# PKU-EPIC/GAPartNet

Hardware: AMD Instinct MI355X
Metric: point-clouds/sec (20k pts, train step) (higher is better)
Workload: dtype f32

## Files before the change

gapartnet_amd/csrc/bn.hip:

```cpp
#include <cstdlib>

#include "bn_stats.h"
#include "gpn_common.h"

namespace {

typedef float f32x4 __attribute__((ext_vector_type(4)));
constexpr int kThreads = 256;
constexpr int kMaxBlocks = 128;


template <int T>
__device__ __forceinline__ double column_total(const double (*red)[T][4], int q, int c, int C4, int R, int part, int P) {
  double acc = 0.0;
  const int cc4 = c >> 2, j = c & 3;
  for (int rr = part; rr < R; rr += P) acc += red[q][rr * C4 + cc4][j];
  for (int off = P >> 1; off >= 1; off >>= 1) acc += __shfl_down(acc, off, P);
  return acc;
}

__host__ __device__ __forceinline__ int sub_lanes(int pairs, int T) {
  int P = 16;
  while (P > 1 && pairs * P > T) P >>= 1;
  return P;
// ... 166 lines not shown
    reinterpret_cast<f32x4*>(y)[t] = v;
  }
}

__global__ void bn_apply_eval_kernel(const gpn::BnFwdPtrs pa, const gpn::BnFwdPtrs pb, int64_t total4, int C4, float eps, int relu,
                                     const int64_t* __restrict__ n_dev) {
  const gpn::BnFwdPtrs& p = blockIdx.y ? pb : pa;
  if (n_dev) total4 = gpn::live_rows(n_dev, total4 / C4) * C4;
  if (blockIdx.x == 0 && p.invstd)
    for (int c = threadIdx.x; c < 4 * C4; c += blockDim.x) p.invstd[c] = 1.0f / sqrtf(p.running_var[c] + eps);
  for (int64_t t = (int64_t)blockIdx.x * blockDim.x + threadIdx.x; t < total4; t += (int64_t)gridDim.x * blockDim.x) {
    const int c4 = (int)(t % C4);
    const f32x4 mu = reinterpret_cast<const f32x4*>(p.running_mean)[c4], var = reinterpret_cast<const f32x4*>(p.running_var)[c4];
    f32x4 is;
#pragma unroll
    for (int j = 0; j < 4; ++j) is[j] = 1.0f / sqrtf(var[j] + eps);
    const f32x4 w = reinterpret_cast<const f32x4*>(p.weight)[c4], b = reinterpret_cast<const f32x4*>(p.bias)[c4];
    f32x4 v = (reinterpret_cast<const f32x4*>(p.x)[t] - mu) * is * w + b;
    if (p.res) v += reinterpret_cast<const f32x4*>(p.res)[t];
    if (relu) {
#pragma unroll
      for (int j = 0; j < 4; ++j) v[j] = v[j] > 0.f ? v[j] : 0.f;
    }
    reinterpret_cast<f32x4*>(p.y)[t] = v;
  }
}

__global__ __launch_bounds__(64) void bn_finalize_bwd_kernel(const double* __restrict__ partial, int blocks, int C,
                                                             float* __restrict__ dweight, float* __restrict__ dbias) {
  const int c = blockIdx.x;
  double s, ss;
  sum_partials(partial, blocks, C, c, s, ss);
  if (threadIdx.x != 0) return;
  dbias[c] = (float)s;
  dweight[c] = (float)ss;
}

__global__ void bn_apply_bwd_kernel(const float* __restrict__ x, const float* __restrict__ y, const float* __restrict__ dy,
                                    const float* __restrict__ mean, const float* __restrict__ invstd,
                                    const float* __restrict__ weight, const float* __restrict__ dweight,
                                    const float* __restrict__ dbias, int64_t total4, int C4, float inv_n, int relu,
                                    int training, float* __restrict__ dx, float* __restrict__ dres) {
  for (int64_t t = (int64_t)blockIdx.x * blockDim.x + threadIdx.x; t < total4; t += (int64_t)gridDim.x * blockDim.x) {
    const int c4 = (int)(t % C4);
    const f32x4 mu = reinterpret_cast<const f32x4*>(mean)[c4], is = reinterpret_cast<const f32x4*>(invstd)[c4];
    const f32x4 w = reinterpret_cast<const f32x4*>(weight)[c4];
    f32x4 g = reinterpret_cast<const f32x4*>(dy)[t];
    if (relu) {
      const f32x4 yv = reinterpret_cast<const f32x4*>(y)[t];
#pragma unroll
      for (int j = 0; j < 4; ++j) g[j] = yv[j] > 0.f ? g[j] : 0.f;
    }
    if (dres) reinterpret_cast<f32x4*>(dres)[t] = g;
    f32x4 v = g;
    if (training) {
      const f32x4 dw = reinterpret_cast<const f32x4*>(dweight)[c4], db = reinterpret_cast<const f32x4*>(dbias)[c4];
      const f32x4 xhat = (reinterpret_cast<const f32x4*>(x)[t] - mu) * is;
      v = g - db * inv_n - xhat * (dw * inv_n);
    }
    reinterpret_cast<f32x4*>(dx)[t] = v * is * w;
  }
}

constexpr int kApplyBatch = 4;

template <bool FIXED>
__global__ __launch_bounds__(kApplyThreads) void bn_apply_fwd_fold_kernel(gpn::BnFwdPtrs pa, gpn::BnFwdPtrs pb, int blocks, int64_t N,
                                                                         int64_t total4, int C4, float eps, float momentum,
                                                                         int relu, const int64_t* __restrict__ n_dev) {
  if (n_dev) {
    N = gpn::live_rows(n_dev, N);
    total4 = N * C4;
    if (N == 0) return;
  }
  const gpn::BnFwdPtrs& pp = blockIdx.y ? pb : pa;
  const float* __restrict__ x = pp.x;
  const float* __restrict__ res = pp.res;
  const void* __restrict__ partial = pp.partial;
  const float* __restrict__ weight = pp.weight;
  const float* __restrict__ bias = pp.bias;
  float* __restrict__ y = pp.y;
  float* __restrict__ mean = pp.mean;
  float* __restrict__ invstd = pp.invstd;
  float* __restrict__ running_mean = pp.running_mean;
  float* __restrict__ running_var = pp.running_var;
  __shared__ double red[2][FIXED ? 1 : kApplyThreads][4];
  __shared__ unsigned long long words[FIXED ? 4 : 1][FIXED ? kFoldMaxC : 1];
  __shared__ double sums[2][kFoldMaxC];
  __shared__ __attribute__((aligned(16))) float stat[4][kFoldMaxC];
  constexpr int U = kApplyBatch;
  const int C = C4 * 4;
  const int64_t stride = (int64_t)gridDim.x * kApplyThreads;
  const int step = (int)(stride % C4);
  int64_t t = (int64_t)blockIdx.x * kApplyThreads + threadIdx.x;
  int c4 = (int)(t % C4);
  f32x4 xv[U], rv[U];
#pragma unroll
  for (int k = 0; k < U; ++k) {
    const int64_t tt = t + k * stride;
    if (tt < total4) {
      xv[k] = reinterpret_cast<const f32x4*>(x)[tt];
      if (res) rv[k] = reinterpret_cast<const f32x4*>(res)[tt];
    }
  }
  if constexpr (FIXED)
    fold_fixed<false>(static_cast<const unsigned long long*>(partial), C, blocks, reinterpret_cast<unsigned long long (*)[kFoldMaxC]>(&words[0][0]), sums);
  else
    fold_partials(static_cast<const double*>(partial), blocks, C4, reinterpret_cast<double (*)[kApplyThreads][4]>(&red[0][0][0]), sums);
  for (int c = threadIdx.x; c < C; c += kApplyThreads) {
    const double m = sums[0][c] / (double)N;
    double var = sums[1][c] / (double)N - m * m;
    if (var < 0.0) var = 0.0;
    const float mu = (float)m, is = (float)(1.0 / sqrt(var + (double)eps));
    stat[0][c] = mu;
    stat[1][c] = is;
    stat[2][c] = weight[c];
    stat[3][c] = bias[c];
    if (blockIdx.x == 0) {
      mean[c] = mu;
      invstd[c] = is;
      if (running_mean) {
        const double unbiased = N > 1 ? var * ((double)N / (double)(N - 1)) : var;
        running_mean[c] = (float)((1.0 - momentum) * running_mean[c] + momentum * m);
        running_var[c] = (float)((1.0 - momentum) * running_var[c] + momentum * unbiased);
      }
    }
  }
  __syncthreads();
  while (true) {
#pragma unroll
    for (int k = 0; k < U; ++k) {
      const int64_t tt = t + k * stride;
      if (tt < total4) {
        const f32x4 mu = reinterpret_cast<const f32x4*>(stat[0])[c4], is = reinterpret_cast<const f32x4*>(stat[1])[c4];
        const f32x4 w = reinterpret_cast<const f32x4*>(stat[2])[c4], b = reinterpret_cast<const f32x4*>(stat[3])[c4];
        f32x4 v = (xv[k] - mu) * is * w + b;
        if (res) v += rv[k];
        if (relu) {
#pragma unroll
          for (int j = 0; j < 4; ++j) v[j] = v[j] > 0.f ? v[j] : 0.f;
        }
        reinterpret_cast<f32x4*>(y)[tt] = v;
      }
      c4 += step;
      c4 = c4 >= C4 ? c4 - C4 : c4;
    }
    t += U * stride;
    if (t >= total4) break;
#pragma unroll
    for (int k = 0; k < U; ++k) {
      const int64_t tt = t + k * stride;
      if (tt < total4) {
        xv[k] = reinterpret_cast<const f32x4*>(x)[tt];
        if (res) rv[k] = reinterpret_cast<const f32x4*>(res)[tt];
      }
    }
  }
}

template <bool FIXED>
__global__ __launch_bounds__(kApplyThreads) void bn_apply_bwd_fold_kernel(gpn::BnBwdPtrs pa, gpn::BnBwdPtrs pb, int blocks, int64_t total4,
                                                                         int C4, float inv_n, int relu, int training,
                                                                         const int64_t* __restrict__ n_dev) {
  if (n_dev) {
    const int64_t N = gpn::live_rows(n_dev, total4 / C4);
    total4 = N * C4;
    inv_n = 1.0f / (float)N;
    if (N == 0) {
      if (blockIdx.x == 0) {
        const gpn::BnBwdPtrs& q = blockIdx.y ? pb : pa;
        for (int c = threadIdx.x; c < C4 * 4; c += kApplyThreads) q.dbias[c] = 0.f, q.dweight[c] = 0.f;
      }
      return;
    }
  }
  const gpn::BnBwdPtrs& pp = blockIdx.y ? pb : pa;
  const float* __restrict__ x = pp.x;
  const float* __restrict__ y = pp.y;
  const float* __restrict__ dy = pp.dy;
  const void* __restrict__ partial = pp.partial;
  const float* __restrict__ mean = pp.mean;
  const float* __restrict__ invstd = pp.invstd;
  const float* __restrict__ weight = pp.weight;
  float* __restrict__ dx = pp.dx;
  float* __restrict__ dres = pp.dres;
  float* __restrict__ dweight = pp.dweight;
  float* __restrict__ dbias = pp.dbias;
  __shared__ double red[2][FIXED ? 1 : kApplyThreads][4];
  __shared__ unsigned long long words[FIXED ? 4 : 1][FIXED ? kFoldMaxC : 1];
  __shared__ double sums[2][kFoldMaxC];
  __shared__ __attribute__((aligned(16))) float stat[5][kFoldMaxC];
  constexpr int U = kApplyBatch;
  const int C = C4 * 4;
  const int64_t stride = (int64_t)gridDim.x * kApplyThreads;
  const int step = (int)(stride % C4);
  int64_t t = (int64_t)blockIdx.x * kApplyThreads + threadIdx.x;
  int c4 = (int)(t % C4);
  f32x4 gv[U], yv[U], xv[U];
#pragma unroll
  for (int k = 0; k < U; ++k) {
    const int64_t tt = t + k * stride;
    if (tt < total4) {
      gv[k] = reinterpret_cast<const f32x4*>(dy)[tt];
      if (relu) yv[k] = reinterpret_cast<const f32x4*>(y)[tt];
      if (training) xv[k] = reinterpret_cast<const f32x4*>(x)[tt];
    }
  }
  if constexpr (FIXED)
    fold_fixed<true>(static_cast<const unsigned long long*>(partial), C, blocks, reinterpret_cast<unsigned long long (*)[kFoldMaxC]>(&words[0][0]), sums);
  else
    fold_partials(static_cast<const double*>(partial), blocks, C4, reinterpret_cast<double (*)[kApplyThreads][4]>(&red[0][0][0]), sums);
  for (int c = threadIdx.x; c < C; c += kApplyThreads) {
    const float db = (float)sums[0][c], dw = (float)sums[1][c];
    stat[0][c] = db;
    stat[1][c] = dw;
    stat[2][c] = mean[c];
    stat[3][c] = invstd[c];
    stat[4][c] = weight[c];
    if (blockIdx.x == 0) {
      dbias[c] = db;
      dweight[c] = dw;
    }
  }
  __syncthreads();
  while (true) {
#pragma unroll
    for (int k = 0; k < U; ++k) {
      const int64_t tt = t + k * stride;
// ... 3 lines not shown
        if (relu) {
#pragma unroll
          for (int j = 0; j < 4; ++j) g[j] = yv[k][j] > 0.f ? g[j] : 0.f;
        }
        if (dres) reinterpret_cast<f32x4*>(dres)[tt] = g;
        f32x4 v = g;
        if (training) {
          const f32x4 db = reinterpret_cast<const f32x4*>(stat[0])[c4], dw = reinterpret_cast<const f32x4*>(stat[1])[c4];
          const f32x4 mu = reinterpret_cast<const f32x4*>(stat[2])[c4];
          const f32x4 xhat = (xv[k] - mu) * is;
          v = g - db * inv_n - xhat * (dw * inv_n);
        }
        reinterpret_cast<f32x4*>(dx)[tt] = v * is * w;
      }
      c4 += step;
      c4 = c4 >= C4 ? c4 - C4 : c4;
    }
    t += U * stride;
    if (t >= total4) break;
#pragma unroll
    for (int k = 0; k < U; ++k) {
      const int64_t tt = t + k * stride;
      if (tt < total4) {
        gv[k] = reinterpret_cast<const f32x4*>(dy)[tt];
        if (relu) yv[k] = reinterpret_cast<const f32x4*>(y)[tt];
        if (training) xv[k] = reinterpret_cast<const f32x4*>(x)[tt];
      }
    }
  }
}

constexpr int kSmallRows = 1024;

template <int CG, int T>
__device__ __forceinline__ void column_sum8(double (&v)[8], double (*scratch)[CG][8] ) {
  constexpr int W = T / 64;
#pragma unroll
  for (int off = 32; off >= CG; off >>= 1) {
#pragma unroll
    for (int q = 0; q < 8; ++q) v[q] += __shfl_down(v[q], off, 64);
  }
  if ((threadIdx.x & 63) < CG) {
#pragma unroll
    for (int q = 0; q < 8; ++q) scratch[threadIdx.x >> 6][threadIdx.x & 63][q] = v[q];
  }
  __syncthreads();
  const int cg = threadIdx.x % CG;
#pragma unroll
  for (int q = 0; q < 8; ++q) {
// ... 104 lines not shown
    reinterpret_cast<f32x4*>(dbias)[c4] = db;
    reinterpret_cast<f32x4*>(dweight)[c4] = dw;
  }
  const f32x4 w = reinterpret_cast<const f32x4*>(weight)[c4];
  const float inv_n = 1.0f / (float)N;
#pragma unroll 8
  for (int row = rl; row < N; row += R) {
    const int64_t t = (int64_t)row * C4 + c4;
    f32x4 g = reinterpret_cast<const f32x4*>(dy)[t];
    if (relu) {
      const f32x4 yv = reinterpret_cast<const f32x4*>(y)[t];
#pragma unroll
      for (int j = 0; j < 4; ++j) g[j] = yv[j] > 0.f ? g[j] : 0.f;
    }
    if (dres) reinterpret_cast<f32x4*>(dres)[t] = g;
    f32x4 v = g;
    if (training) {
      const f32x4 xhat = (reinterpret_cast<const f32x4*>(x)[t] - mu) * is;
      v = g - db * inv_n - xhat * (dw * inv_n);
    }
    reinterpret_cast<f32x4*>(dx)[t] = v * is * w;
  }
}

int reduce_blocks(int64_t N, int C4) {
  const int R = kReduceThreads / C4;
  int64_t b = gpn::cdiv(N, (int64_t)R * 2);
  if (b > kMaxBlocks) b = kMaxBlocks;
  if (b < 1) b = 1;
  return (int)b;
}

int fold_grid(int64_t total4) {
  int64_t g = gpn::cdiv(total4, (int64_t)kApplyThreads);
  if (g > 320) g = 320;
  return (int)(g < 1 ? 1 : g);
}

constexpr size_t kReduceLds = (size_t)2 * kReduceThreads * 4 * sizeof(double);

int apply_grid(int64_t total4) {
  int64_t g = gpn::cdiv(total4, kThreads);
  if (g > 4096) g = 4096;
  return (int)(g < 1 ? 1 : g);
}

// ... 144 lines not shown
  hipLaunchKernelGGL(bn_finalize_bwd_kernel, dim3(C), dim3(64), 0, stream, partial, blocks, C,
                     dweight, dbias);
  GPN_CHECK_LAUNCH();
  hipLaunchKernelGGL(bn_apply_bwd_kernel, dim3(apply_grid(total4)), dim3(kThreads), 0, stream, x, y, dy, mean, invstd,
                     weight, dweight, dbias, total4, C4, 1.0f / (float)N, relu, training, dx, dres);
  GPN_CHECK_LAUNCH();
  return GPN_OK;
}

bool gpn::bn_two_pass(int64_t N, int C) { return N >= 1 && C % 4 == 0 && C <= kFoldMaxC; }

int gpn::bn_fwd_train_fused(const gpn::BnFwdPtrs& p, const gpn::BnFwdPtrs* twin, int64_t N, int C, float eps, float momentum,
                            int relu, hipStream_t stream, const gpn::DevRows& rows) {
  for (const gpn::BnFwdPtrs* q : {&p, twin}) {
    if (!q) continue;
    GPN_CHECK_ARG(q->x && q->weight && q->bias && q->y && q->mean && q->invstd && q->partial);
    GPN_CHECK_ARG((q->running_mean == nullptr) == (q->running_var == nullptr));
  }
  GPN_CHECK_ARG(gpn::bn_two_pass(N, C));
  GPN_CHECK_ARG(!twin || (twin->res == nullptr) == (p.res == nullptr));
  const int64_t total4 = N * (C / 4);
  gpn::ProfScope prof(GPN_K_BN, stream, 0.0, 4.0 * (double)N * C * (p.res ? 3 : 2) * (twin ? 2 : 1), rows.dev, N);
  const int64_t Np = gpn::plan_rows(N, rows);
  hipLaunchKernelGGL(bn_apply_fwd_fold_kernel<true>, dim3(fold_grid(Np * (C / 4)), twin ? 2 : 1), dim3(kApplyThreads), 0, stream, p,
                     twin ? *twin : p, gpn::stat_slot_count(Np), N, total4, C / 4, eps, momentum, relu, rows.dev);
  GPN_CHECK_LAUNCH();
  return GPN_OK;
}

int gpn::bn_bwd_fused(const gpn::BnBwdPtrs& p, const gpn::BnBwdPtrs* twin, int64_t N, int C, int relu, int training,
                      hipStream_t stream, const gpn::DevRows& rows) {
  for (const gpn::BnBwdPtrs* q : {&p, twin}) {
    if (!q) continue;
    GPN_CHECK_ARG(q->x && q->dy && q->weight && q->mean && q->invstd && q->dx && q->dweight && q->dbias && q->partial && (q->y || !relu));
  }
  GPN_CHECK_ARG(gpn::bn_two_pass(N, C));
  GPN_CHECK_ARG(!twin || (twin->dres == nullptr) == (p.dres == nullptr));
  const int64_t total4 = N * (C / 4);
  gpn::ProfScope prof(GPN_K_BN, stream, 0.0, 4.0 * (double)N * C * (4 + (p.dres ? 1 : 0)) * (twin ? 2 : 1), rows.dev, N);
  const int64_t Np = gpn::plan_rows(N, rows);
  hipLaunchKernelGGL(bn_apply_bwd_fold_kernel<true>, dim3(fold_grid(Np * (C / 4)), twin ? 2 : 1), dim3(kApplyThreads), 0, stream, p,
                     twin ? *twin : p, gpn::stat_slot_count(Np), total4, C / 4, 1.0f / (float)N, relu, training, rows.dev);
  GPN_CHECK_LAUNCH();
  return GPN_OK;
}
```

gapartnet_amd/csrc/gpn_common.h:

```cpp
#pragma once
#include <cstdlib>
#include <cstring>
#include <hip/hip_runtime.h>

#include <cstdint>
#include <cstdio>

#include "../../include/gpn.h"

namespace gpn {

void set_error(const char* fmt, ...);

struct ProfScope {
  int id;
  hipStream_t stream;
  hipEvent_t start = nullptr;
  int64_t tag = 0;
  ProfScope(int kernel_id, hipStream_t s, double flops, double bytes, int64_t tag = 0);
  ProfScope(int kernel_id, hipStream_t s, double flops, double bytes, const int64_t* rows_dev, int64_t bound, int64_t tag = 0);
  ~ProfScope();
};
inline int64_t prof_shape_tag(int K, int64_t n_dst, int cin, int cout, bool twin) {
  return ((int64_t)(twin ? 1 : 0) << 62) | ((int64_t)(K & 63) << 48) | ((int64_t)((cin / 16) & 255) << 40) |
// ... 88 lines not shown
  float mu, is, w, b;
};
__device__ __forceinline__ AffineCol affine_col(const ConvAffine& ep, uint32_t col) {
  return AffineCol{ep.mean[col], 1.0f / sqrtf(ep.var[col] + ep.eps), ep.weight[col], ep.bias[col]};
}
__device__ __forceinline__ float affine_apply(const ConvAffine& ep, const AffineCol& c, float v, uint32_t e) {
  v = (v - c.mu) * c.is * c.w + c.b;
  if (ep.res) v += ep.res[e];
  if (ep.relu) v = v > 0.f ? v : 0.f;
  return v;
}
#endif
struct BnFwdPtrs {
  const float* x = nullptr;
  const float* res = nullptr;
  const void* partial = nullptr;
  const float* weight = nullptr;
  const float* bias = nullptr;
  float* y = nullptr;
  float* mean = nullptr;
  float* invstd = nullptr;
  float* running_mean = nullptr;
  float* running_var = nullptr;
};
struct BnBwdPtrs {
  const float* x = nullptr;
  const float* y = nullptr;
  const float* dy = nullptr;
  const void* partial = nullptr;
  const float* mean = nullptr;
  const float* invstd = nullptr;
  const float* weight = nullptr;
  float* dx = nullptr;
  float* dres = nullptr;
  float* dweight = nullptr;
  float* dbias = nullptr;
};
inline size_t stat_slab_bytes(int C) { return align_up((size_t)kStatSlots * 4 * C * sizeof(unsigned long long)); }

int spconv_fwd_into(const float* in, const float* packed_w, const int32_t* nbr, const int32_t* nbr_p, const int32_t* perm, int K,
                    int64_t n_dst, int cin, int cout, float* out, int accumulate, const ConvStats& stats, void* ws,
                    size_t ws_bytes, hipStream_t stream, const DevRows& rows = DevRows());
struct ConvRoute {
  enum Kind { kNone, kTiles, kMsplit, kDirect, kLockstep, kUnroutable };
  Kind kind = kNone;
  bool sums = false;
  bool affine = false;
  size_t ws_bytes = 0;
};
ConvRoute spconv_fwd_route(int K, int64_t n_dst, int cin, int cout, const DevRows& rows = DevRows());
struct PackBf16Desc {
  const float* W;
  uint16_t* packed;
  int K, cin, cout, oki;
};
int spconv_bf16_check(const char* who, int K, int64_t n_dst, int cin, int cout);
int spconv_bf16_launch(const uint16_t* in, const uint16_t* packed, const int32_t* nbr, const int32_t* nbr_p, const int32_t* perm,
                       int K, int64_t n_dst, int cin, int cout, const gpn_conv_epilogue_bf16_t* ep, void* out, hipStream_t stream);
int pack_bf16_many(const PackBf16Desc* descs, int n, hipStream_t stream);
// ... 12 lines not shown
struct WgradSets {
  int n = 0;
  WgradSet s[kWgradSets];
};
struct WgradReduceJob {
  const float* partial;
  float* dW;
  int64_t elems;
  int S, K, cin, cout, oki, few;
};
int wgrad_slices(int K, int cin, int cout, int64_t n_dst);
int wgrad_contract(const WgradSets& sets, int K, int64_t n_dst, int cin, int cout, int S, hipStream_t stream,
                   const int64_t* n_dst_dev = nullptr);
WgradReduceJob wgrad_reduce_job(const float* partial, int S, int K, int cin, int cout, int flags, float* dW);
int wgrad_reduce_many(const WgradReduceJob* jobs, int n, hipStream_t stream);
int rulebook_level_counts_dev(const int32_t* indices, int64_t n_max, const int64_t* n_dev, int64_t batch_size,
                              const int64_t* max_coord_dev, int n_levels, int64_t* counts, void* ws, size_t ws_bytes,
                              hipStream_t stream);
bool bn_two_pass(int64_t N, int C);
int bn_fwd_train_fused(const BnFwdPtrs& p, const BnFwdPtrs* twin, int64_t N, int C, float eps, float momentum, int relu,
                       hipStream_t stream, const DevRows& rows = DevRows());
int bn_bwd_fused(const BnBwdPtrs& p, const BnBwdPtrs* twin, int64_t N, int C, int relu, int training, hipStream_t stream,
                 const DevRows& rows = DevRows());
int bn_fwd_train_rows(const float* x, const float* res, const float* weight, const float* bias, int64_t N, const DevRows& rows,
                      int C, float eps, float momentum, int relu, float* y, float* mean, float* invstd, float* running_mean,
                      float* running_var, void* ws, size_t ws_bytes, hipStream_t stream);
int bn_fwd_eval_rows(const float* x, const float* res, const float* weight, const float* bias, const float* mean,
                     const float* invstd, int64_t N, const DevRows& rows, int C, int relu, float* y, hipStream_t stream);
int bn_fwd_eval_running(const BnFwdPtrs& pa, const BnFwdPtrs* pb, int64_t N, const DevRows& rows, int C, float eps, int relu,
                        hipStream_t stream);
int bn_bwd_rows(const float* x, const float* y, const float* dy, const float* weight, const float* mean, const float* invstd,
                int64_t N, const DevRows& rows, int C, int relu, int training, float* dx, float* dres, float* dweight,
                float* dbias, void* ws, size_t ws_bytes, hipStream_t stream);

}

#define GPN_CHECK_ARG(cond)                                                     \
  do {                                                                          \
    if (!(cond)) {                                                              \
      gpn::set_error("%s: bad argument: %s", __func__, #cond);                  \
      return GPN_ERR_ARG;                                                       \
    }                                                                           \
  } while (0)

#define GPN_CHECK_HIP(expr)                                                     \
  do {                                                                          \
// ... 24 lines not shown
```

gapartnet_amd/csrc/net.hip:

```cpp
#include <unistd.h>

#include <cstdlib>

#include <algorithm>
#include <atomic>
#include <condition_variable>
#include <mutex>
#include <string>
#include <thread>
#include <vector>

#include "gpn_common.h"
#include "spconv_pack.h"

namespace {

constexpr int kThreads = 256;

std::atomic<int> g_bn_fusion{1};

struct ConcatPtrs {
  const float4* a;
  const float4* b;
  float4* dst;
// ... 308 lines not shown
  }
  const bool pair = n_nets == 2;
  std::vector<char> folded(n_ops, 0);
  if (inference && g_bn_fusion.load(std::memory_order_relaxed)) {
    std::vector<int> readers(n_slots, 0);
    for (int i = 0; i < n_ops; ++i) {
      readers[ops[i].src0]++;
      if (ops[i].src1 >= 0) readers[ops[i].src1]++;
    }
    for (int i = 0; i + 1 < n_ops; ++i) {
      const gpn_net_op_t &cv_op = ops[i], &bn_op = ops[i + 1];
      if (cv_op.kind != GPN_NET_CONV || bn_op.kind != GPN_NET_BN || bn_op.src0 != cv_op.dst || readers[cv_op.dst] != 1) continue;
      if (bn_op.src1 == cv_op.dst || bn_op.dst == cv_op.src0) continue;
      const gpn_net_rulebook_t& rb = rbs[cv_op.rulebook];
      const gpn_net_conv_t& cv = nets[0].convs[cv_op.param];
      bool ok = gpn::spconv_fwd_route(rb.K, rb.n_dst, cv.cin, cv.cout, dev_rows(nets[0].slots[cv_op.dst])).affine;
      for (int t = 0; t < n_nets; ++t) {
        const gpn_net_bn_t& bn = nets[t].bns[bn_op.param];
        ok = ok && bn.running_mean && bn.running_var && bn.eps == nets[0].bns[bn_op.param].eps;
      }
      if (ok) folded[i + 1] = 1;
    }
  }
  for (int i = 0; i < n_ops; ++i) {
    const gpn_net_op_t& op = ops[i];
    if (folded[i]) continue;
    for (int t = 0; t < n_nets; ++t)
      if (!nets[t].slots[op.src0].data || !nets[t].slots[op.dst].data) {
        gpn::set_error("%s: op %d: null activation pointer", who, i);
        return GPN_ERR_ARG;
      }
    const gpn_net_slot_t &s0 = nets[0].slots[op.src0], &d = nets[0].slots[op.dst];
    if (op.kind == GPN_NET_CONV) {
      const gpn_net_rulebook_t& rb = rbs[op.rulebook];
      const gpn_net_conv_t& cv = nets[0].convs[op.param];
      gpn::ConvStats st;
      st.slab = slab_of[0][i];
      st.slot_mask = gpn::stat_slot_count(plan_of(d)) - 1;
      if (pair) {
        st.twin.in = nets[1].slots[op.src0].data;
        st.twin.packed = packed_of[1][i];
        st.twin.out = nets[1].slots[op.dst].data;
        st.twin.slab = slab_of[1][i];
      }
      float* out = d.data;
      if (i + 1 < n_ops && folded[i + 1]) {
        const gpn_net_op_t& bo = ops[i + 1];
        auto affine = [&](int t) {
          const gpn_net_bn_t& bn = nets[t].bns[bo.param];
// ... 8 lines not shown
            gpn::set_error("%s: op %d: null activation pointer", who, i + 1);
            return GPN_ERR_ARG;
          }
        st.ep = affine(0);
        out = nets[0].slots[bo.dst].data;
        if (pair) {
          st.twin.ep = affine(1);
          st.twin.out = nets[1].slots[bo.dst].data;
        }
      }
      rc = gpn::spconv_fwd_into(s0.data, packed_of[0][i], rb.nbr, rb.nbr_p, rb.perm, rb.K, rb.n_dst, cv.cin, cv.cout, out, 0, st,
                                op_ws, op_ws_bytes, stream, dev_rows(d));
    } else if (op.kind == GPN_NET_BN) {
      const int relu = (op.flags & GPN_NET_RELU) ? 1 : 0;
      gpn::BnFwdPtrs pp[2];
      for (int t = 0; t < n_nets; ++t) {
        const gpn_net_bn_t& bn = nets[t].bns[op.param];
        pp[t].x = nets[t].slots[op.src0].data;
        pp[t].res = op.src1 >= 0 ? nets[t].slots[op.src1].data : nullptr;
        pp[t].partial = slab_of[t][i];
        pp[t].weight = bn.weight, pp[t].bias = bn.bias, pp[t].y = nets[t].slots[op.dst].data;
        pp[t].mean = bn.save_mean, pp[t].invstd = bn.save_invstd;
        pp[t].running_mean = bn.running_mean, pp[t].running_var = bn.running_var;
      }
      const gpn_net_bn_t& bn0 = nets[0].bns[op.param];
      const bool together = pair && nets[1].bns[op.param].eps == bn0.eps && nets[1].bns[op.param].momentum == bn0.momentum;
      if (training && slab_of[0][i] && together) {
        rc = gpn::bn_fwd_train_fused(pp[0], &pp[1], s0.rows, bn0.C, bn0.eps, bn0.momentum, relu, stream, dev_rows(s0));
      } else if (!training) {
        for (int t = 0; t < n_nets; ++t)
          if (!nets[t].bns[op.param].running_mean || !nets[t].bns[op.param].running_var) {
            gpn::set_error("%s: op %d: eval-mode BatchNorm needs running statistics", who, i);
            return GPN_ERR_ARG;
          }
        if (together) {
          rc = gpn::bn_fwd_eval_running(pp[0], &pp[1], s0.rows, dev_rows(s0), bn0.C, bn0.eps, relu, stream);
        } else {
          for (int t = 0; t < n_nets && rc == GPN_OK; ++t)
            rc = gpn::bn_fwd_eval_running(pp[t], nullptr, s0.rows, dev_rows(s0), nets[t].bns[op.param].C, nets[t].bns[op.param].eps, relu, stream);
        }
      } else {
        for (int t = 0; t < n_nets && rc == GPN_OK; ++t) {
          const gpn_net_bn_t& bn = nets[t].bns[op.param];
          if (training && slab_of[t][i]) {
            rc = gpn::bn_fwd_train_fused(pp[t], nullptr, s0.rows, bn.C, bn.eps, bn.momentum, relu, stream, dev_rows(s0));
          } else {
// ... 273 lines not shown
  }
  const Need need = workspace_need(ops, n_ops, nets[0].slots, rbs, nets[0].convs);
  const size_t per_net = need.tmp + need.packed + need.stats;
  const size_t total_need = n_nets * per_net + need.op + n_nets * need.wgrad;
  if (!ws || ws_bytes < total_need) {
    gpn::set_error("%s: workspace too small (%zu needed, %zu given)", who, total_need, ws_bytes);
    return GPN_ERR_WS;
  }
  char* base = static_cast<char*>(ws);
  float* tmp[2] = {reinterpret_cast<float*>(base), reinterpret_cast<float*>(base + per_net)};
  void* op_ws = base + n_nets * per_net;
  const size_t op_ws_bytes = need.op;
  void* wgrad_ws = base + n_nets * per_net + need.op;
  const size_t wgrad_ws_bytes = ws_bytes - (n_nets * per_net + need.op);
  std::vector<const float*> packed_of[2];
  for (int t = 0; t < n_nets; ++t) {
    rc = pack_program(ops, n_ops, rbs, nets[t].convs, true, base + t * per_net + need.tmp, packed_of[t], stream);
    if (rc) return rc;
  }
  std::vector<unsigned long long*> bn_slab[2];
  for (int t = 0; t < n_nets; ++t) bn_slab[t].assign(n_ops, nullptr);
  std::vector<int> fused_by(n_ops, -1);
  std::vector<char> sums_done(n_ops, 0);
  if (g_bn_fusion.load(std::memory_order_relaxed)) {
    std::vector<int> first_reader(n_slots, -1), producer(n_slots, -1);
    for (int i = n_ops - 1; i >= 0; --i) {
      first_reader[ops[i].src0] = i;
      if (ops[i].src1 >= 0) first_reader[ops[i].src1] = i;
      producer[ops[i].dst] = i;
    }
    size_t off = 0;
    for (int i = 0; i < n_ops; ++i) {
      if (ops[i].kind != GPN_NET_CONV) continue;
      const int j = producer[ops[i].src0];
      if (j < 0 || ops[j].kind != GPN_NET_BN || first_reader[ops[i].src0] != i) continue;
      if (ops[i].src0 == 0 && !need_input_grad) continue;
      const gpn_net_rulebook_t& rb = rbs[ops[i].rulebook];
      const gpn_net_conv_t& cv = nets[0].convs[ops[i].param];
      const gpn_net_slot_t& in_slot = nets[0].slots[ops[i].src0];
      if (!gpn::bn_two_pass(plan_of(in_slot), cv.cin) ||
          !gpn::spconv_fwd_route(rb.K, rb.n_src, cv.cout, cv.cin, dev_rows(in_slot)).sums)
        continue;
      for (int t = 0; t < n_nets; ++t)
        bn_slab[t][j] = reinterpret_cast<unsigned long long*>(base + t * per_net + need.tmp + need.packed + off);
      off += gpn::stat_slab_bytes(cv.cin);
      fused_by[i] = j;
    }
    if (off)
      for (int t = 0; t < n_nets; ++t) GPN_CHECK_HIP(hipMemsetAsync(base + t * per_net + need.tmp + need.packed, 0, off, stream));
  }
  SideStream* side = side_stream();
  if (!side) {
    gpn::set_error("%s: could not create the weight-gradient stream", who);
    return GPN_ERR_HIP;
  }
  GPN_CHECK_HIP(hipEventRecord(side->join, side->stream));
  GPN_CHECK_HIP(hipStreamWaitEvent(stream, side->join, 0));
  bool forked = false;
  int device = 0;
  GPN_CHECK_HIP(hipGetDevice(&device));
  GPN_CHECK_ARG(device >= 0 && device < gpn::kMaxDevices);
  DeviceWorker& dw = device_worker(device);
  std::lock_guard<std::mutex> pass_lock(dw.pass_mu);
  WgradWorker& worker = dw.worker;
  worker.begin(device, side->stream, wgrad_ws, wgrad_ws_bytes, (size_t)n_ops * n_nets);
  struct PassGuard {
    WgradWorker& w;
    bool closed = false;
    ~PassGuard() {
// ... 85 lines not shown
        const gpn_net_bn_t& bn = nets[t].bns[op.param];
        gpn_net_slot_t& ts0 = nets[t].slots[op.src0];
        if (!ts0.grad || !bn.dweight || !bn.dbias) {
          gpn::set_error("%s: op %d: null gradient buffer", who, i);
          return GPN_ERR_ARG;
        }
        GradTarget tx = grad_target(ts0, tmp[t]);
        if (tx.staged) {
          gpn::set_error("%s: op %d: BatchNorm input consumed twice is not supported", who, i);
          return GPN_ERR_ARG;
        }
        if (op.src1 >= 0 && (op.src1 != 0 || need_input_grad)) {
          if (!nets[t].slots[op.src1].grad) {
            gpn::set_error("%s: op %d: null residual gradient buffer", who, i);
            return GPN_ERR_ARG;
          }
          tr[t] = grad_target(nets[t].slots[op.src1], tmp[t]);
        }
        pp[t].x = ts0.data, pp[t].y = nets[t].slots[op.dst].data, pp[t].dy = nets[t].slots[op.dst].grad;
        pp[t].partial = bn_slab[t][i];
        pp[t].mean = training ? bn.save_mean : bn.running_mean;
        pp[t].invstd = bn.save_invstd, pp[t].weight = bn.weight;
        pp[t].dx = tx.ptr, pp[t].dres = tr[t].ptr, pp[t].dweight = bn.dweight, pp[t].dbias = bn.dbias;
      }
      const gpn_net_bn_t& bn0 = nets[0].bns[op.param];
      if (sums_done[i] && pair) {
        rc = gpn::bn_bwd_fused(pp[0], &pp[1], s0.rows, bn0.C, relu, training ? 1 : 0, stream, dev_rows(s0));
      } else {
        for (int t = 0; t < n_nets && rc == GPN_OK; ++t) {
          if (sums_done[i])
            rc = gpn::bn_bwd_fused(pp[t], nullptr, s0.rows, bn0.C, relu, training ? 1 : 0, stream, dev_rows(s0));
          else
            rc = gpn::bn_bwd_rows(pp[t].x, pp[t].y, pp[t].dy, pp[t].weight, pp[t].mean, pp[t].invstd, s0.rows, dev_rows(s0), bn0.C, relu,
                                  training ? 1 : 0, pp[t].dx, pp[t].dres, pp[t].dweight, pp[t].dbias, op_ws, op_ws_bytes, stream);
        }
      }
      if (rc) return rc;
      for (int t = 0; t < n_nets; ++t) {
        nets[t].slots[op.src0].grad_state = 1;
        if (pp[t].dres) {
          rc = commit(nets[t].slots[op.src1], tr[t], stream);
          if (rc) return rc;
        }
      }
    } else {
      gpn_net_slot_t& s1 = nets[0].slots[op.src1];
      for (int t = 0; t < n_nets; ++t)
        if (!nets[t].slots[op.src0].grad || !nets[t].slots[op.src1].grad) {
          gpn::set_error("%s: op %d: null gradient buffer", who, i);
          return GPN_ERR_ARG;
        }
      SplitPtrs sa{(const float4*)d.grad, (float4*)s0.grad, (float4*)s1.grad}, sb = sa;
      if (pair)
        sb = SplitPtrs{(const float4*)nets[1].slots[op.dst].grad, (float4*)nets[1].slots[op.src0].grad,
                       (float4*)nets[1].slots[op.src1].grad};
      hipLaunchKernelGGL(split_kernel, dim3(grid_for(plan_of(d) * (d.channels / 4)), n_nets), dim3(kThreads), 0, stream, sa, sb, d.rows,
                         s0.channels / 4, s1.channels / 4, s0.grad_state, s1.grad_state, d.rows_dev);
      GPN_CHECK_LAUNCH();
      for (int t = 0; t < n_nets; ++t) nets[t].slots[op.src0].grad_state = nets[t].slots[op.src1].grad_state = 1;
    }
  }
  std::string worker_err;
  guard.closed = true;
  rc = worker.finish(worker_err);
  if (rc) {
    gpn::set_error("%s", worker_err.c_str());
    return rc;
  }
  if (forked) {
    GPN_CHECK_HIP(hipEventRecord(side->join, side->stream));
    GPN_CHECK_HIP(hipStreamWaitEvent(stream, side->join, 0));
  }
  return GPN_OK;
}
// ... 207 lines not shown
```

Before: 1049.

## Fuse BatchNorm outputs into concat buffers and fuse split with BN backward stats

In training, a BatchNorm whose output feeds a concat now writes straight into the concat buffer with a strided store, so the concat copy is skipped. In backward, a new joint kernel reads the concat gradient in place. It accumulates the BN dbias/dweight statistics for the left half and copies the right half's gradient out, replacing the separate split pass. The fused BN apply kernels then read dy and y strided from the concat buffers. This removes extra full-tensor read/write passes, at the cost of strided addressing, more template variants and more planning logic in the net executor.

Result: no change. 1053 (median of 4 runs) (+0.4%).

```diff
diff --git a/gapartnet_amd/csrc/bn.hip b/gapartnet_amd/csrc/bn.hip
--- a/gapartnet_amd/csrc/bn.hip
+++ b/gapartnet_amd/csrc/bn.hip
@@ -212,7 +212,13 @@
 #pragma unroll
       for (int j = 0; j < 4; ++j) v[j] = v[j] > 0.f ? v[j] : 0.f;
     }
-    reinterpret_cast<f32x4*>(p.y)[t] = v;
+    if (!p.ldy && !p.y2) {
+      reinterpret_cast<f32x4*>(p.y)[t] = v;
+    } else {
+      const int64_t row = t / C4;
+      reinterpret_cast<f32x4*>(p.y)[row * (p.ldy ? p.ldy >> 2 : C4) + c4] = v;
+      if (p.y2) reinterpret_cast<f32x4*>(p.y2)[row * (p.ldy2 >> 2) + c4] = v;
+    }
   }
 }
 
@@ -254,7 +260,7 @@
 
 constexpr int kApplyBatch = 4;
 
-template <bool FIXED>
+template <bool FIXED, bool STRIDED = false>
 __global__ __launch_bounds__(kApplyThreads) void bn_apply_fwd_fold_kernel(gpn::BnFwdPtrs pa, gpn::BnFwdPtrs pb, int blocks, int64_t N,
                                                                          int64_t total4, int C4, float eps, float momentum,
                                                                          int relu, const int64_t* __restrict__ n_dev) {
@@ -270,6 +276,8 @@
   const float* __restrict__ weight = pp.weight;
   const float* __restrict__ bias = pp.bias;
   float* __restrict__ y = pp.y;
+  float* __restrict__ y2 = STRIDED ? pp.y2 : nullptr;
+  const int ldy4 = pp.ldy ? pp.ldy >> 2 : C4, ldy2_4 = pp.ldy2 >> 2;
   float* __restrict__ mean = pp.mean;
   float* __restrict__ invstd = pp.invstd;
   float* __restrict__ running_mean = pp.running_mean;
@@ -284,6 +292,8 @@
   const int step = (int)(stride % C4);
   int64_t t = (int64_t)blockIdx.x * kApplyThreads + threadIdx.x;
   int c4 = (int)(t % C4);
+  int64_t row = STRIDED ? t / C4 : 0;
+  const int64_t row_step = STRIDED ? stride / C4 : 0;
   f32x4 xv[U], rv[U];
 #pragma unroll
   for (int k = 0; k < U; ++k) {
@@ -330,9 +340,15 @@
 #pragma unroll
           for (int j = 0; j < 4; ++j) v[j] = v[j] > 0.f ? v[j] : 0.f;
         }
-        reinterpret_cast<f32x4*>(y)[tt] = v;
+        if constexpr (STRIDED) {
+          reinterpret_cast<f32x4*>(y)[row * ldy4 + c4] = v;
+          if (y2) reinterpret_cast<f32x4*>(y2)[row * ldy2_4 + c4] = v;
+        } else {
+          reinterpret_cast<f32x4*>(y)[tt] = v;
+        }
       }
       c4 += step;
+      if constexpr (STRIDED) row += row_step + (c4 >= C4 ? 1 : 0);
       c4 = c4 >= C4 ? c4 - C4 : c4;
     }
     t += U * stride;
@@ -348,7 +364,7 @@
   }
 }
 
-template <bool FIXED>
+template <bool FIXED, bool STRIDED = false>
 __global__ __launch_bounds__(kApplyThreads) void bn_apply_bwd_fold_kernel(gpn::BnBwdPtrs pa, gpn::BnBwdPtrs pb, int blocks, int64_t total4,
                                                                          int C4, float inv_n, int relu, int training,
                                                                          const int64_t* __restrict__ n_dev) {
@@ -368,6 +384,7 @@
   const float* __restrict__ x = pp.x;
   const float* __restrict__ y = pp.y;
   const float* __restrict__ dy = pp.dy;
+  const int lddy4 = pp.lddy ? pp.lddy >> 2 : C4, ldy4 = pp.ldy ? pp.ldy >> 2 : C4;
   const void* __restrict__ partial = pp.partial;
   const float* __restrict__ mean = pp.mean;
   const float* __restrict__ invstd = pp.invstd;
@@ -386,14 +403,22 @@
   const int step = (int)(stride % C4);
   int64_t t = (int64_t)blockIdx.x * kApplyThreads + threadIdx.x;
   int c4 = (int)(t % C4);
+  const int64_t row_step = STRIDED ? stride / C4 : 0;
+  int64_t lr = STRIDED ? t / C4 : 0;
+  int lc = c4;
   f32x4 gv[U], yv[U], xv[U];
 #pragma unroll
   for (int k = 0; k < U; ++k) {
     const int64_t tt = t + k * stride;
     if (tt < total4) {
-      gv[k] = reinterpret_cast<const f32x4*>(dy)[tt];
-      if (relu) yv[k] = reinterpret_cast<const f32x4*>(y)[tt];
+      gv[k] = reinterpret_cast<const f32x4*>(dy)[STRIDED ? lr * lddy4 + lc : tt];
+      if (relu) yv[k] = reinterpret_cast<const f32x4*>(y)[STRIDED ? lr * ldy4 + lc : tt];
       if (training) xv[k] = reinterpret_cast<const f32x4*>(x)[tt];
+    }
+    if constexpr (STRIDED) {
+      lc += step;
+      lr += row_step + (lc >= C4 ? 1 : 0);
+      lc = lc >= C4 ? lc - C4 : lc;
     }
   }
   if constexpr (FIXED)
@@ -443,9 +468,14 @@
     for (int k = 0; k < U; ++k) {
       const int64_t tt = t + k * stride;
       if (tt < total4) {
-        gv[k] = reinterpret_cast<const f32x4*>(dy)[tt];
-        if (relu) yv[k] = reinterpret_cast<const f32x4*>(y)[tt];
+        gv[k] = reinterpret_cast<const f32x4*>(dy)[STRIDED ? lr * lddy4 + lc : tt];
+        if (relu) yv[k] = reinterpret_cast<const f32x4*>(y)[STRIDED ? lr * ldy4 + lc : tt];
         if (training) xv[k] = reinterpret_cast<const f32x4*>(x)[tt];
+      }
+      if constexpr (STRIDED) {
+        lc += step;
+        lr += row_step + (lc >= C4 ? 1 : 0);
+        lc = lc >= C4 ? lc - C4 : lc;
       }
     }
   }
@@ -596,6 +626,85 @@
     reinterpret_cast<f32x4*>(dx)[t] = v * is * w;
   }
 }
+
+constexpr int kJointThreads = 256;
+constexpr int kJointRows = 4;
+
+__global__ __launch_bounds__(kJointThreads) void bn_joint_stats_kernel(gpn::BnJointPtrs pa, gpn::BnJointPtrs pb, int64_t N, int C4,
+                                                                       int ldg4, int ldy4, int cb4, int acc, int slot_mask,
+                                                                       const int64_t* __restrict__ n_dev) {
+  N = gpn::live_rows(n_dev, N);
+  const gpn::BnJointPtrs& pp = blockIdx.y ? pb : pa;
+  const f32x4* __restrict__ g = reinterpret_cast<const f32x4*>(pp.g);
+  const f32x4* __restrict__ y = reinterpret_cast<const f32x4*>(pp.y);
+  const f32x4* __restrict__ x = reinterpret_cast<const f32x4*>(pp.x);
+  f32x4* __restrict__ db = reinterpret_cast<f32x4*>(pp.db);
+  __shared__ __attribute__((aligned(16))) double red[2][kJointThreads][4];
+  constexpr int T = kJointThreads;
+  const int C = C4 * 4, R = T / C4;
+  const int r = threadIdx.x / C4, c4 = threadIdx.x - r * C4;
+  const bool lane_ok = r < R;
+  f32x4 mu = {0.f, 0.f, 0.f, 0.f}, is = {0.f, 0.f, 0.f, 0.f};
+  if (lane_ok) {
+    mu = reinterpret_cast<const f32x4*>(pp.mean)[c4];
+    is = reinterpret_cast<const f32x4*>(pp.invstd)[c4];
+  }
+  const int64_t block_rows = (int64_t)R * kJointRows;
+  const int64_t n_blocks = (N + block_rows - 1) / block_rows;
+  const int P = sub_lanes(2 * C, T);
+  const int part = threadIdx.x % P;
+  for (int64_t b = blockIdx.x; b < n_blocks; b += gridDim.x) {
+    const int64_t row0 = b * block_rows + r;
+    f32x4 gv[kJointRows], yv[kJointRows], xv[kJointRows];
+#pragma unroll
+    for (int k = 0; k < kJointRows; ++k) {
+      const int64_t row = row0 + (int64_t)k * R;
+      if (lane_ok && row < N) {
+        gv[k] = g[row * ldg4 + c4];
+        if (y) yv[k] = y[row * ldy4 + c4];
+        xv[k] = x[row * C4 + c4];
+      }
+    }
+    if (db && lane_ok) {
+      for (int c = c4; c < cb4; c += C4) {
+#pragma unroll
+        for (int k = 0; k < kJointRows; ++k) {
+          const int64_t row = row0 + (int64_t)k * R;
+          if (row < N) {
+            f32x4 v = g[row * ldg4 + C4 + c];
+            if (acc) v += db[row * cb4 + c];
+            db[row * cb4 + c] = v;
+          }
+        }
+      }
+    }
+    double s[8] = {0.0, 0.0, 0.0, 0.0, 0.0, 0.0, 0.0, 0.0};
+#pragma unroll
+    for (int k = 0; k < kJointRows; ++k) {
+      if (lane_ok && row0 + (int64_t)k * R < N) {
+#pragma unroll
+        for (int j = 0; j < 4; ++j) {
+          const float gm = (y && !(yv[k][j] > 0.f)) ? 0.f : gv[k][j];
+          s[j] += (double)gm;
+          s[4 + j] += (double)gm * (double)((xv[k][j] - mu[j]) * is[j]);
+        }
+      }
+    }
+#pragma unroll
+    for (int j = 0; j < 4; ++j) red[0][threadIdx.x][j] = s[j], red[1][threadIdx.x][j] = s[4 + j];
+    __syncthreads();
+    for (int e = threadIdx.x / P; e < 2 * C; e += T / P) {
+      const int q = e / C, c = e - q * C;
+      const double total = column_total<T>(red, q, c, C4, R, part, P);
+      if (part == 0) {
+        gpn::stat_add<true>(pp.slab, C, (int)(b & slot_mask), c, 2 * q, total, total);
+        gpn::stat_add<true>(pp.slab, C, (int)(b & slot_mask), c, 2 * q + 1, total, total);
+      }
+    }
+    __syncthreads();
+  }
+}
+
 
 int reduce_blocks(int64_t N, int C4) {
   const int R = kReduceThreads / C4;
@@ -786,8 +895,16 @@
   const int64_t total4 = N * (C / 4);
   gpn::ProfScope prof(GPN_K_BN, stream, 0.0, 4.0 * (double)N * C * (p.res ? 3 : 2) * (twin ? 2 : 1), rows.dev, N);
   const int64_t Np = gpn::plan_rows(N, rows);
-  hipLaunchKernelGGL(bn_apply_fwd_fold_kernel<true>, dim3(fold_grid(Np * (C / 4)), twin ? 2 : 1), dim3(kApplyThreads), 0, stream, p,
-                     twin ? *twin : p, gpn::stat_slot_count(Np), N, total4, C / 4, eps, momentum, relu, rows.dev);
+  const bool strided = p.ldy || p.y2 || (twin && (twin->ldy || twin->y2));
+  for (const gpn::BnFwdPtrs* q : {&p, twin})
+    if (q) GPN_CHECK_ARG(q->ldy % 4 == 0 && (!q->ldy || q->ldy >= C) && (!q->y2 || (q->ldy2 % 4 == 0 && q->ldy2 >= C)));
+  const dim3 grid(fold_grid(Np * (C / 4)), twin ? 2 : 1);
+  if (strided)
+    hipLaunchKernelGGL((bn_apply_fwd_fold_kernel<true, true>), grid, dim3(kApplyThreads), 0, stream, p, twin ? *twin : p,
+                       gpn::stat_slot_count(Np), N, total4, C / 4, eps, momentum, relu, rows.dev);
+  else
+    hipLaunchKernelGGL((bn_apply_fwd_fold_kernel<true>), grid, dim3(kApplyThreads), 0, stream, p, twin ? *twin : p,
+                       gpn::stat_slot_count(Np), N, total4, C / 4, eps, momentum, relu, rows.dev);
   GPN_CHECK_LAUNCH();
   return GPN_OK;
 }
@@ -803,8 +920,35 @@
   const int64_t total4 = N * (C / 4);
   gpn::ProfScope prof(GPN_K_BN, stream, 0.0, 4.0 * (double)N * C * (4 + (p.dres ? 1 : 0)) * (twin ? 2 : 1), rows.dev, N);
   const int64_t Np = gpn::plan_rows(N, rows);
-  hipLaunchKernelGGL(bn_apply_bwd_fold_kernel<true>, dim3(fold_grid(Np * (C / 4)), twin ? 2 : 1), dim3(kApplyThreads), 0, stream, p,
-                     twin ? *twin : p, gpn::stat_slot_count(Np), total4, C / 4, 1.0f / (float)N, relu, training, rows.dev);
+  const bool strided = p.lddy || p.ldy || (twin && (twin->lddy || twin->ldy));
+  for (const gpn::BnBwdPtrs* q : {&p, twin})
+    if (q) GPN_CHECK_ARG(q->lddy % 4 == 0 && q->ldy % 4 == 0 && (!q->lddy || q->lddy >= C) && (!q->ldy || q->ldy >= C));
+  const dim3 grid(fold_grid(Np * (C / 4)), twin ? 2 : 1);
+  if (strided)
+    hipLaunchKernelGGL((bn_apply_bwd_fold_kernel<true, true>), grid, dim3(kApplyThreads), 0, stream, p, twin ? *twin : p,
+                       gpn::stat_slot_count(Np), total4, C / 4, 1.0f / (float)N, relu, training, rows.dev);
+  else
+    hipLaunchKernelGGL((bn_apply_bwd_fold_kernel<true>), grid, dim3(kApplyThreads), 0, stream, p, twin ? *twin : p,
+                       gpn::stat_slot_count(Np), total4, C / 4, 1.0f / (float)N, relu, training, rows.dev);
   GPN_CHECK_LAUNCH();
   return GPN_OK;
 }
+
+int gpn::bn_bwd_joint_stats(const gpn::BnJointPtrs& p, const gpn::BnJointPtrs* twin, int64_t N, int C, int ldg, int ldy, int cb,
+                            int acc, hipStream_t stream, const gpn::DevRows& rows) {
+  for (const gpn::BnJointPtrs* q : {&p, twin}) {
+    if (!q) continue;
+    GPN_CHECK_ARG(q->g && q->x && q->mean && q->invstd && q->slab && (q->db || !cb));
+  }
+  GPN_CHECK_ARG(gpn::bn_two_pass(N, C));
+  GPN_CHECK_ARG(cb >= 0 && cb % 4 == 0 && ldg % 4 == 0 && ldg >= C + cb && (!p.y || (ldy % 4 == 0 && ldy >= C)));
+  GPN_CHECK_ARG(!twin || (twin->y == nullptr) == (p.y == nullptr));
+  const int64_t Np = gpn::plan_rows(N, rows);
+  gpn::ProfScope prof(GPN_K_BN, stream, 0.0, 4.0 * (double)N * ((p.y ? 3 : 2) * C + (acc ? 3 : 2) * cb) * (twin ? 2 : 1), rows.dev, N);
+  int64_t grid = gpn::cdiv(Np, (int64_t)(kJointThreads / (C / 4)) * kJointRows);
+  grid = grid < 1 ? 1 : (grid > 4096 ? 4096 : grid);
+  hipLaunchKernelGGL(bn_joint_stats_kernel, dim3((unsigned)grid, twin ? 2 : 1), dim3(kJointThreads), 0, stream, p, twin ? *twin : p, N,
+                     C / 4, ldg / 4, ldy / 4, cb / 4, acc, gpn::stat_slot_count(Np) - 1, rows.dev);
+  GPN_CHECK_LAUNCH();
+  return GPN_OK;
+}
diff --git a/gapartnet_amd/csrc/gpn_common.h b/gapartnet_amd/csrc/gpn_common.h
--- a/gapartnet_amd/csrc/gpn_common.h
+++ b/gapartnet_amd/csrc/gpn_common.h
@@ -134,6 +134,9 @@
   float* invstd = nullptr;
   float* running_mean = nullptr;
   float* running_var = nullptr;
+  int ldy = 0;
+  float* y2 = nullptr;
+  int ldy2 = 0;
 };
 struct BnBwdPtrs {
   const float* x = nullptr;
@@ -147,6 +150,17 @@
   float* dres = nullptr;
   float* dweight = nullptr;
   float* dbias = nullptr;
+  int lddy = 0;
+  int ldy = 0;
+};
+struct BnJointPtrs {
+  const float* g = nullptr;
+  const float* y = nullptr;
+  const float* x = nullptr;
+  const float* mean = nullptr;
+  const float* invstd = nullptr;
+  unsigned long long* slab = nullptr;
+  float* db = nullptr;
 };
 inline size_t stat_slab_bytes(int C) { return align_up((size_t)kStatSlots * 4 * C * sizeof(unsigned long long)); }
 
@@ -205,6 +219,8 @@
                        hipStream_t stream, const DevRows& rows = DevRows());
 int bn_bwd_fused(const BnBwdPtrs& p, const BnBwdPtrs* twin, int64_t N, int C, int relu, int training, hipStream_t stream,
                  const DevRows& rows = DevRows());
+int bn_bwd_joint_stats(const BnJointPtrs& p, const BnJointPtrs* twin, int64_t N, int C, int ldg, int ldy, int cb, int acc,
+                       hipStream_t stream, const DevRows& rows = DevRows());
 int bn_fwd_train_rows(const float* x, const float* res, const float* weight, const float* bias, int64_t N, const DevRows& rows,
                       int C, float eps, float momentum, int relu, float* y, float* mean, float* invstd, float* running_mean,
                       float* running_var, void* ws, size_t ws_bytes, hipStream_t stream);
diff --git a/gapartnet_amd/csrc/net.hip b/gapartnet_amd/csrc/net.hip
--- a/gapartnet_amd/csrc/net.hip
+++ b/gapartnet_amd/csrc/net.hip
@@ -354,9 +354,31 @@
       if (ok) folded[i + 1] = 1;
     }
   }
+  std::vector<int> cat_of[2];
+  cat_of[0].assign(n_ops, -1), cat_of[1].assign(n_ops, -1);
+  std::vector<char> cat_direct(n_ops, 0);
+  if (!inference && g_bn_fusion.load(std::memory_order_relaxed)) {
+    std::vector<int> readers(n_slots, 0), producer(n_slots, -1);
+    for (int i = 0; i < n_ops; ++i) {
+      readers[ops[i].src0]++;
+      if (ops[i].src1 >= 0) readers[ops[i].src1]++;
+      producer[ops[i].dst] = i;
+    }
+    for (int k = 0; k < n_ops; ++k) {
+      if (ops[k].kind != GPN_NET_CONCAT) continue;
+      const int u = producer[ops[k].src0], s = producer[ops[k].src1];
+      if (u < 0 || s < 0 || u >= k || s >= k || u == s || ops[u].kind != GPN_NET_BN || ops[s].kind != GPN_NET_BN) continue;
+      if (readers[ops[k].src0] != 1 || cat_of[1][s] >= 0 || cat_of[0][s] >= 0 || cat_of[1][u] >= 0) continue;
+      bool ok = true;
+      for (int t = 0; t < n_nets; ++t) ok = ok && (!training || (slab_of[t][u] && slab_of[t][s]));
+      if (!ok) continue;
+      cat_of[0][u] = k, cat_of[1][s] = k, cat_direct[k] = 1;
+    }
+  }
   for (int i = 0; i < n_ops; ++i) {
     const gpn_net_op_t& op = ops[i];
     if (folded[i]) continue;
+    if (cat_direct[i]) continue;
     for (int t = 0; t < n_nets; ++t)
       if (!nets[t].slots[op.src0].data || !nets[t].slots[op.dst].data) {
         gpn::set_error("%s: op %d: null activation pointer", who, i);
@@ -411,6 +433,20 @@
         pp[t].weight = bn.weight, pp[t].bias = bn.bias, pp[t].y = nets[t].slots[op.dst].data;
         pp[t].mean = bn.save_mean, pp[t].invstd = bn.save_invstd;
         pp[t].running_mean = bn.running_mean, pp[t].running_var = bn.running_var;
+        for (int half = 0; half < 2; ++half) {
+          if (cat_of[half][i] < 0) continue;
+          const gpn_net_op_t& co = ops[cat_of[half][i]];
+          float* cat = nets[t].slots[co.dst].data;
+          if (!cat) {
+            gpn::set_error("%s: op %d: null activation pointer", who, cat_of[half][i]);
+            return GPN_ERR_ARG;
+          }
+          const int ld = nets[0].slots[co.dst].channels;
+          if (half == 0)
+            pp[t].y = cat, pp[t].ldy = ld;
+          else
+            pp[t].y2 = cat + nets[0].slots[co.src0].channels, pp[t].ldy2 = ld;
+        }
       }
       const gpn_net_bn_t& bn0 = nets[0].bns[op.param];
       const bool together = pair && nets[1].bns[op.param].eps == bn0.eps && nets[1].bns[op.param].momentum == bn0.momentum;
@@ -730,6 +766,7 @@
   for (int t = 0; t < n_nets; ++t) bn_slab[t].assign(n_ops, nullptr);
   std::vector<int> fused_by(n_ops, -1);
   std::vector<char> sums_done(n_ops, 0);
+  std::vector<int> joint_cat(n_ops, -1), joint_bn(n_ops, -1);
   if (g_bn_fusion.load(std::memory_order_relaxed)) {
     std::vector<int> first_reader(n_slots, -1), producer(n_slots, -1);
     for (int i = n_ops - 1; i >= 0; --i) {
@@ -753,6 +790,22 @@
         bn_slab[t][j] = reinterpret_cast<unsigned long long*>(base + t * per_net + need.tmp + need.packed + off);
       off += gpn::stat_slab_bytes(cv.cin);
       fused_by[i] = j;
+    }
+    std::vector<int> readers(n_slots, 0);
+    for (int i = 0; i < n_ops; ++i) {
+      readers[ops[i].src0]++;
+      if (ops[i].src1 >= 0) readers[ops[i].src1]++;
+    }
+    for (int k = 0; k < n_ops; ++k) {
+      if (ops[k].kind != GPN_NET_CONCAT) continue;
+      const int u = producer[ops[k].src0];
+      if (u < 0 || u >= k || ops[u].kind != GPN_NET_BN || readers[ops[k].src0] != 1 || bn_slab[0][u] || joint_cat[u] >= 0) continue;
+      const gpn_net_slot_t& left = nets[0].slots[ops[k].src0];
+      if (!gpn::bn_two_pass(plan_of(left), left.channels)) continue;
+      for (int t = 0; t < n_nets; ++t)
+        bn_slab[t][u] = reinterpret_cast<unsigned long long*>(base + t * per_net + need.tmp + need.packed + off);
+      off += gpn::stat_slab_bytes(left.channels);
+      joint_cat[u] = k, joint_bn[k] = u;
     }
     if (off)
       for (int t = 0; t < n_nets; ++t) GPN_CHECK_HIP(hipMemsetAsync(base + t * per_net + need.tmp + need.packed, 0, off, stream));
@@ -884,6 +937,11 @@
         pp[t].mean = training ? bn.save_mean : bn.running_mean;
         pp[t].invstd = bn.save_invstd, pp[t].weight = bn.weight;
         pp[t].dx = tx.ptr, pp[t].dres = tr[t].ptr, pp[t].dweight = bn.dweight, pp[t].dbias = bn.dbias;
+        if (joint_cat[i] >= 0 && sums_done[i]) {
+          const gpn_net_slot_t& cat = nets[t].slots[ops[joint_cat[i]].dst];
+          pp[t].dy = cat.grad, pp[t].lddy = cat.channels;
+          pp[t].y = cat.data, pp[t].ldy = cat.channels;
+        }
       }
       const gpn_net_bn_t& bn0 = nets[0].bns[op.param];
       if (sums_done[i] && pair) {
@@ -912,6 +970,30 @@
           gpn::set_error("%s: op %d: null gradient buffer", who, i);
           return GPN_ERR_ARG;
         }
+      if (joint_bn[i] >= 0) {
+        const gpn_net_op_t& bo = ops[joint_bn[i]];
+        gpn::BnJointPtrs jp[2];
+        for (int t = 0; t < n_nets; ++t) {
+          const gpn_net_bn_t& bn = nets[t].bns[bo.param];
+          jp[t].g = nets[t].slots[op.dst].grad;
+          jp[t].y = (bo.flags & GPN_NET_RELU) ? nets[t].slots[op.dst].data : nullptr;
+          jp[t].x = nets[t].slots[bo.src0].data;
+          jp[t].mean = training ? bn.save_mean : bn.running_mean;
+          jp[t].invstd = bn.save_invstd;
+          jp[t].slab = bn_slab[t][joint_bn[i]];
+          jp[t].db = nets[t].slots[op.src1].grad;
+          if (!jp[t].x || !jp[t].mean || !jp[t].invstd) {
+            gpn::set_error("%s: op %d: null BatchNorm input / statistics pointer", who, joint_bn[i]);
+            return GPN_ERR_ARG;
+          }
+        }
+        rc = gpn::bn_bwd_joint_stats(jp[0], pair ? &jp[1] : nullptr, d.rows, s0.channels, d.channels, d.channels, s1.channels,
+                                     s1.grad_state, stream, dev_rows(d));
+        if (rc) return rc;
+        sums_done[joint_bn[i]] = 1;
+        for (int t = 0; t < n_nets; ++t) nets[t].slots[op.src0].grad_state = nets[t].slots[op.src1].grad_state = 1;
+        continue;
+      }
       SplitPtrs sa{(const float4*)d.grad, (float4*)s0.grad, (float4*)s1.grad}, sb = sa;
       if (pair)
         sb = SplitPtrs{(const float4*)nets[1].slots[op.dst].grad, (float4*)nets[1].slots[op.src0].grad,
```
